# gevaertlab/sequoia-pub

Hardware: AMD Instinct MI355X
Metric: slides/sec (1000-patch WSI, UNI-dim, 20k-gene head) (higher is better)
Workload: dtype f16x3; 1 GPU; pipeline: 1000 x 224x224 uint8 patches/slide -> ResNet-50 embed -> k-Means(100) -> ViS(D=2048, depth 6, 16 heads, G=20820) forward (BASELINE config 3), patches uploaded from pinned host memory every step; embedder=ResNet-50 (src/resnet.py forward_extract), feature_dim=2048, patch_size=224, parallelism=slide-sharded x1

## Files before the change

### sequoia-pub_amd/csrc/chain_x3.hip

```cpp
#include "gemm.h"
#include "x3_fmt.h"

#include <cstdio>
#include <cstdlib>
#include <type_traits>

extern int g_dbg;

namespace {

constexpr uint32_t OOB = 0x80000000u;
typedef __attribute__((address_space(3))) void lds_void;

__device__ __forceinline__ void glds16(__amdgpu_buffer_rsrc_t rsrc, char* lds_base, uint32_t voffset) {
    __builtin_amdgcn_raw_ptr_buffer_load_lds(rsrc, (lds_void*)lds_base, 16, voffset, 0, 0, 0);
}
__device__ __forceinline__ u32x4 lds128(const char* p) { return *reinterpret_cast<const u32x4*>(p); }
template <int N> __device__ __forceinline__ void wait_vm() { asm volatile("s_waitcnt vmcnt(%0)" ::"n"(N) : "memory"); }
__device__ __forceinline__ void wait_vm_n(int n) {
    switch (n) {
        case 0: wait_vm<0>(); break;
        case 2: wait_vm<2>(); break;
        case 4: wait_vm<4>(); break;
        case 6: wait_vm<6>(); break;
// ... 11 lines not shown
constexpr int B_PLANE = N1 * 64;
constexpr int KT_BYTES = 2 * A_PLANE + 2 * B_PLANE;
constexpr int LDS_BYTES = 2 * KT_BYTES;
constexpr int YROW = N1 * 4;

struct ChainX3Args {
    const uint16_t* t2; long long plT2;
    const uint16_t* w3; const uint16_t* w1n; long long plW;
    const float* b3; const float* cs3; const float* b1n; const float* cs1n;
    const uint16_t* res; long long plRes;
    uint16_t* y; long long plY;
    uint16_t* t1n; long long plT1n;
    int P;
    uint32_t t2_bytes, w3_bytes;
    const uint16_t* xin; long long plX;
    const uint16_t* wd;
    const float* bd; const float* csd;
    uint32_t wd_bytes;
    const uint16_t* t1; long long plT1;
    const uint16_t* w2;
    const float* b2; const float* cs2;
    uint32_t w2_bytes;
    int W, HW;
    int dbg;
    int xcd_walk;
};

template <int N2, bool F16, bool DS, bool TAIL, bool WIDE = false>
__global__ __launch_bounds__(256, 2) void chain_x3_kernel(const ChainX3Args p) {
    using Fmt = X3Fmt<F16>;
    extern __shared__ __attribute__((aligned(16))) char smem[];
    const int tid = threadIdx.x, lane = tid & 63;
    const int wave = __builtin_amdgcn_readfirstlane(tid >> 6);
    const int l31 = lane & 31, lh = lane >> 5;

    const auto rsTh = __builtin_amdgcn_make_buffer_rsrc((void*)p.t2, 0, (int)p.t2_bytes, 0x00020000);
    const auto rsTl = __builtin_amdgcn_make_buffer_rsrc((void*)(p.t2 + p.plT2), 0, (int)p.t2_bytes, 0x00020000);
    const auto rsXh = __builtin_amdgcn_make_buffer_rsrc((void*)(DS ? p.xin : p.t2), 0, (int)p.t2_bytes, 0x00020000);
    const auto rsXl = __builtin_amdgcn_make_buffer_rsrc((void*)(DS ? p.xin + p.plX : p.t2 + p.plT2), 0, (int)p.t2_bytes, 0x00020000);

    constexpr int NI2 = N2 == 64 ? 1 : 2;
    const int pi = N2 == 64 ? wave >> 1 : 0, cj = N2 == 64 ? wave & 1 : wave;
    const uint16_t* const w1src = p.w1n + (size_t)cj * 16 * 512 + lane * 8;
    constexpr int W1PRE = DS ? 4 : 3;
    u32x4 wbh[4][4], wbl[4][4];
    auto load_w1 = [&](int g, int slot) {
// ... 231 lines not shown
                    const uint32_t h = Fmt::pack2(d0, d1);
                    const uint32_t l = Fmt::rest2(d0, d1, h);
                    acc[i][j][r] = x3_relu((s3 * acc[i][j][r] + b3) + Fmt::sum_lo(h, l));
                    acc[i][j][r + 1] = x3_relu((s3 * acc[i][j][r + 1] + b3) + Fmt::sum_hi(h, l));
                }
        }
    }
    __syncthreads();

#pragma unroll
    for (int i = 0; i < 2; ++i)
#pragma unroll
        for (int j = 0; j < 2; ++j)
#pragma unroll
            for (int r = 0; r < 16; ++r) {
                const int row = i * 32 + (r & 3) + 8 * (r >> 2) + 4 * lh;
                const int col = wave * 64 + j * 32 + l31;
                *reinterpret_cast<float*>(smem + row * YROW + ((((col >> 3) ^ (row & 31))) << 5) + (col & 7) * 4) = acc[i][j][r];
            }
#pragma unroll
    for (int g = 0; g < W1PRE; ++g) load_w1(g, g);
    __syncthreads();
    {
#pragma unroll
        for (int u = 0; u < 8; ++u) {
            const int row = u * 8 + rsub;
            const int m = p0 + row;
            char* chunk = smem + row * YROW + ((c8 ^ (row & 31)) << 5);
            const f32x4 a0 = *reinterpret_cast<const f32x4*>(chunk), a1 = *reinterpret_cast<const f32x4*>(chunk + 16);
            float v[8] = {a0[0], a0[1], a0[2], a0[3], a1[0], a1[1], a1[2], a1[3]};
            if constexpr (!DS) {
                float idn[8];
                x3_join8<F16>(rh[u], rl[u], idn);
#pragma unroll
                for (int e = 0; e < 8; ++e) v[e] = x3_relu((scale8[e] * v[e] + bias8[e]) + idn[e]);
            }
            u32x4 hi, lo;
            x3_split8<F16>(v, hi, lo);
            *reinterpret_cast<u32x4*>(chunk) = hi;
            *reinterpret_cast<u32x4*>(chunk + 16) = lo;
            if (m < p.P && !(p.dbg & 1)) {
                u32x4* qh = reinterpret_cast<u32x4*>(p.y + (size_t)m * N1 + c8 * 8);
                u32x4* ql = reinterpret_cast<u32x4*>(p.y + p.plY + (size_t)m * N1 + c8 * 8);
                *qh = hi; *ql = lo;
            }
        }
    }
    __syncthreads();

    f32x16 acc2[NI2];
#pragma unroll
    for (int i = 0; i < NI2; ++i)
#pragma unroll
        for (int e = 0; e < 16; ++e) acc2[i][e] = 0.f;
    if (!(p.dbg & 8))
#pragma unroll
    for (int g = 0; g < 4; ++g) {
        if (g == 0)
#pragma unroll
            for (int g2 = W1PRE; g2 < 4; ++g2) load_w1(g2, g2);
#pragma unroll
        for (int s4 = 0; s4 < 4; ++s4) {
            const int s = g * 4 + s4;
            u32x4 ah[NI2], al[NI2];
#pragma unroll
            for (int i = 0; i < NI2; ++i) {
// ... 62 lines not shown
        const bool d = e0 >= FRAG_WD;
        const int r = e0 - (d ? FRAG_WD : 0), q = r >> 9, lane = (r & 511) >> 3;
        const uint16_t* w = d ? wd : w3;
        if (w) src = at(w, (q >> 2) * 32 + (lane & 31), (q & 3) * 16 + (lane >> 5) * 8, N1, K1);
    } else if (e0 < FRAG_WD) {
        const int r = e0 - FRAG_W1, q = r >> 9, lane = (r & 511) >> 3;
        if ((q >> 4) * 32 < n2) src = at(w1n, (q >> 4) * 32 + (lane & 31), (q & 15) * 16 + (lane >> 5) * 8, n2, N1);
    } else if (w2) {
        const int r = e0 - FRAG_W2, g = r >> 11, n = (r & 2047) >> 5, kk = r & 31;
        const int cb = g / 9, tap = g - cb * 9;
        src = at(w2, n, tap * 64 + cb * 32 + kk, 64, 576);
    }
    if (src) *reinterpret_cast<u32x4*>(dst + (size_t)pl * FRAG + e0) = *reinterpret_cast<const u32x4*>(src + (size_t)pl * plSrc);
}

}

size_t sq_chain_x3_frag_bytes() { return (size_t)2 * FRAG * 2; }

int sq_launch_chain_x3_c64(int f16, const uint16_t* t2, long long plT2, const uint16_t* res, long long plRes, uint16_t* y, long long plY,
                           uint16_t* t1n, long long plT1n, int n2, const uint16_t* w3, const uint16_t* w1n, long long plW, size_t w3_bytes,
                           const float* b3, const float* cs3, const float* b1n, const float* cs1n,
                           const uint16_t* xin, long long plX, const uint16_t* wd, size_t wd_bytes, const float* bd, const float* csd,
                           const uint16_t* t1, long long plT1, const uint16_t* w2, size_t w2_bytes, const float* b2, const float* cs2, int W, int HW,
                           long long P, uint16_t* frag, int w_tiled, hipStream_t stream) {
    SQ_REQUIRE(n2 == 64 || n2 == 128, "chain_x3: next width %d (64 or 128)", n2);
    SQ_REQUIRE(P > 0 && P * N1 * 2 < (1ll << 31), "chain_x3: %lld pixels exceed the 2 GiB descriptor limit", P);
    const bool tail = t1 != nullptr;
    SQ_REQUIRE((t2 || tail) && y && t1n && w3 && w1n && b3 && b1n && frag && w3_bytes >= (size_t)N1 * K1 * 2, "chain_x3: null pointer / weight extent");
    SQ_REQUIRE(!tail || (w2 && b2 && w2_bytes >= (size_t)64 * 576 * 2 && W >= 3 && W <= 70 && HW >= W && HW % W == 0 && P % HW == 0),
               "chain_x3: tail form needs the 3x3 weights and maps up to 70 wide (W=%d, HW=%d)", W, HW);
    const bool wide = tail && W > 62;
    const bool ds = res == nullptr;
    SQ_REQUIRE(!ds || (xin && wd && bd && wd_bytes >= (size_t)N1 * K1 * 2), "chain_x3: neither an identity tensor nor a downsample branch");
    ChainX3Args a;
    hipLaunchKernelGGL(chain_x3_pack_kernel, dim3((2 * (FRAG / 8) + 255) / 256), dim3(256), 0, stream, w3, w1n, ds ? wd : nullptr,
                       tail ? w2 : nullptr, plW, n2, w_tiled, frag);
    SQ_LAUNCH_CHECK();
    a.t2 = t2; a.plT2 = plT2; a.w3 = frag; a.w1n = frag + FRAG_W1; a.plW = FRAG; a.b3 = b3; a.cs3 = cs3; a.b1n = b1n; a.cs1n = cs1n;
    a.res = res; a.plRes = plRes; a.y = y; a.plY = plY; a.t1n = t1n; a.plT1n = plT1n; a.P = (int)P;
    a.t2_bytes = (uint32_t)(P * K1 * 2);
    auto clamp = [](size_t b) { return (uint32_t)(b < 0x7fffffffu ? b : 0x7fffffffu); };
    a.w3_bytes = clamp(w3_bytes);
    a.xin = xin; a.plX = plX; a.wd = frag + FRAG_WD; a.bd = bd; a.csd = csd; a.wd_bytes = clamp(wd_bytes);
    a.t1 = t1; a.plT1 = plT1; a.w2 = frag + FRAG_W2; a.b2 = b2; a.cs2 = cs2; a.w2_bytes = (uint32_t)((FRAG - FRAG_W2) * 2); a.W = W; a.HW = HW; a.dbg = g_dbg;
    { const char* e = getenv("SQ_X3_TAIL_XCD_WALK"); a.xcd_walk = tail ? (e ? atoi(e) : 64) : 0; }
    using I64 = std::integral_constant<int, 64>; using I128 = std::integral_constant<int, 128>;
    using T = std::true_type; using F = std::false_type;
    auto pick_tail = [&](auto n2c, auto f16c, auto dsc) {
        return wide ? (const void*)chain_x3_kernel<decltype(n2c)::value, decltype(f16c)::value, decltype(dsc)::value, true, true>
             : tail ? (const void*)chain_x3_kernel<decltype(n2c)::value, decltype(f16c)::value, decltype(dsc)::value, true>
                    : (const void*)chain_x3_kernel<decltype(n2c)::value, decltype(f16c)::value, decltype(dsc)::value, false>;
    };
    auto pick_ds = [&](auto n2c, auto f16c) { return ds ? pick_tail(n2c, f16c, T{}) : pick_tail(n2c, f16c, F{}); };
    auto pick_f16 = [&](auto n2c) { return f16 ? pick_ds(n2c, T{}) : pick_ds(n2c, F{}); };
    const void* fn = n2 == 64 ? pick_f16(I64{}) : pick_f16(I128{});
    SQ_HIP_CHECK(hipFuncSetAttribute(fn, hipFuncAttributeMaxDynamicSharedMemorySize, LDS_BYTES));
    int prof = -1;
    if (sq_prof_on()) {
        char name[96];
        snprintf(name, sizeof(name), "%s_%s_c64_cn%d%s_P%lld", tail ? "tail" : "chain", f16 ? "f16x3" : "bf16x3", n2, ds ? "_ds" : "", P);
        prof = sq_prof_begin(name, 2.0 * P * ((tail ? 576.0 * 64 : 0.0) + 64.0 * 256 * (ds ? 2 : 1) + 256.0 * n2), (double)P * 4.0 * (64 + (ds ? 64 : 256) + 256 + n2), stream);
    }
    const dim3 grid((unsigned)((P + PX - 1) / PX)), block(256);
    void* kargs[] = {(void*)&a};
    SQ_HIP_CHECK(hipLaunchKernel(fn, grid, block, kargs, LDS_BYTES, stream));
    if (prof >= 0) sq_prof_end(prof, stream);
    return SQ_OK;
}

extern "C" int sq_dbg_chain_x3(int f16, int n2, int ds, int tail, long long P, int W, void* act, void* wts, void* fp, void* frag, void* stream) {
    uint16_t* a = (uint16_t*)act;
    const uint16_t* w = (const uint16_t*)wts;
    const float* f = (const float*)fp;
    uint16_t* t1 = a; uint16_t* res = t1 + 2 * P * 64; uint16_t* y = res + 2 * P * 256; uint16_t* t1n = y + 2 * P * 256;
    const long long plW = 102400;
    return sq_launch_chain_x3_c64(f16, tail ? nullptr : t1, P * 64, ds ? nullptr : res, P * 256, y, P * 256, t1n, P * 128, n2,
                                  w, w + 16384, plW, (size_t)(plW * 2), f, f + 256, f + 512, f + 640,
                                  ds ? t1 : nullptr, P * 64, ds ? w + 49152 : nullptr, (size_t)(plW - 49152) * 2, ds ? f + 768 : nullptr, ds ? f + 1024 : nullptr,
                                  tail ? t1 : nullptr, P * 64, tail ? w + 65536 : nullptr, (size_t)(plW - 65536) * 2, tail ? f + 1280 : nullptr,
                                  tail ? f + 1344 : nullptr, W, W * W, P, (uint16_t*)frag, 0, (hipStream_t)stream);
}
```

### sequoia-pub_amd/csrc/chain_x3w.hip

```cpp
#include "gemm.h"
#include "x3_fmt.h"

#include <cstdio>
#include <cstdlib>
#include <type_traits>

extern int g_dbg;

namespace {

constexpr uint32_t OOB = 0x80000000u;
typedef __attribute__((address_space(3))) void lds_void;

__device__ __forceinline__ void glds16(__amdgpu_buffer_rsrc_t rsrc, char* lds_base, uint32_t voffset) {
    __builtin_amdgcn_raw_ptr_buffer_load_lds(rsrc, (lds_void*)lds_base, 16, voffset, 0, 0, 0);
}
__device__ __forceinline__ void glds16_nt(__amdgpu_buffer_rsrc_t rsrc, char* lds_base, uint32_t voffset) {
    __builtin_amdgcn_raw_ptr_buffer_load_lds(rsrc, (lds_void*)lds_base, 16, voffset, 0, 0, 2);
}
__device__ __forceinline__ u32x4 lds128(const char* p) { return *reinterpret_cast<const u32x4*>(p); }
__device__ __forceinline__ u32x2 lds64(const char* p) { return *reinterpret_cast<const u32x2*>(p); }
__device__ __forceinline__ void st_lds64(char* p, u32x2 v) { *reinterpret_cast<u32x2*>(p) = v; }
template <int N> __device__ __forceinline__ void wait_vm() { asm volatile("s_waitcnt vmcnt(%0)" ::"n"(N) : "memory"); }
__device__ __forceinline__ void wait_vm_n(int n) {
    switch (n >> 1) {
        case 0: wait_vm<0>(); break;
        case 1: wait_vm<2>(); break;
        case 2: wait_vm<4>(); break;
        case 3: wait_vm<6>(); break;
        case 4: wait_vm<8>(); break;
        case 5: wait_vm<10>(); break;
        case 6: wait_vm<12>(); break;
        case 7: wait_vm<14>(); break;
        default: wait_vm<16>(); break;
    }
}

struct ChainWArgs {
    const uint16_t* t2; long long plT2;
    const uint16_t* res; long long plRes;
    uint16_t* y; long long plY;
    uint16_t* t1n; long long plT1n;
    const uint16_t* w3; const uint16_t* w1n; long long plW;
    const float* b3; const float* cs3; const float* b1n; const float* cs1n;
    int P, tiles, tiled;
    uint32_t w3_bytes, w1n_bytes;
    int dbg;
};

template <int C, int N2_> struct ChainWCfg {
    static constexpr int N2 = N2_, N1 = 4 * C, NS = N1 / 32, KS1 = C / 16, NT2 = N2 / 32;
    static constexpr int H = N2 / 128;
    static constexpr int KSH = KS1 / H;
    static constexpr int KTL = C / H / 32;
    static constexpr int W3R = KTL / 2;
    static constexpr int NW3 = 2 * W3R;
    static constexpr int STEPS = H * NS + H;
    static constexpr int T = 512, PX = 128;
    static constexpr int UNIT = 16384, UH = 8192;
    static constexpr int RING = 6 * UNIT;
    static constexpr int XYW = 4096;
    static constexpr int XY = 4 * 3 * XYW;
    static constexpr int BIAS_FLOATS = 2 * N1 + 2 * N2;
    static constexpr int LDS_BYTES = RING + XY + BIAS_FLOATS * 4;
    static_assert((C == 128 && (N2 == 128 || N2 == 256)) || (C == 256 && N2 == 256), "C -> next width: 128 -> 128 | 256 (28 x 28 stage), 256 -> 256 (14 x 14 stage)");
    static_assert(32 * (C / H) * 4 <= UNIT && N2 * (32 / H) * 4 == UNIT && KTL >= 2, "unit sizes");
    static_assert(32 * N2 * 2 * 4 <= RING, "t1' staging (one plane per pixel group) must fit the dead ring");
};
// ... 169 lines not shown
#pragma unroll
                    for (int g = 0; g < 4; ++g) {
                        char* a = xrow + ((g ^ swz) << 4) + 8 * lh;
                        const int cb = s * 32 + 8 * g + 4 * lh;
                        const f32x4 b = *reinterpret_cast<const f32x4*>(BS + cb), sc = *reinterpret_cast<const f32x4*>(BS + N1 + cb);
                        const u32x2 ih = lds64(a), il = lds64(a + 2048);
                        float v[4];
                        v[0] = x3_relu((sc[0] * accy[4 * g + 0] + b[0]) + Fmt::sum_lo(ih[0], il[0]));
                        v[1] = x3_relu((sc[1] * accy[4 * g + 1] + b[1]) + Fmt::sum_hi(ih[0], il[0]));
                        v[2] = x3_relu((sc[2] * accy[4 * g + 2] + b[2]) + Fmt::sum_lo(ih[1], il[1]));
                        v[3] = x3_relu((sc[3] * accy[4 * g + 3] + b[3]) + Fmt::sum_hi(ih[1], il[1]));
                        const uint32_t h0 = Fmt::pack2(v[0], v[1]), h1 = Fmt::pack2(v[2], v[3]);
                        const uint32_t l0 = Fmt::rest2(v[0], v[1], h0);
                        const uint32_t l1 = Fmt::rest2(v[2], v[3], h1);
                        st_lds64(a, u32x2{h0, h1});
                        st_lds64(a + 2048, u32x2{l0, l1});
                    }
                }
                asm volatile("s_waitcnt lgkmcnt(0)" ::: "memory");
                __builtin_amdgcn_s_barrier();
            }
        }
    } else {
        const uint32_t act_bytes = (uint32_t)p.P * N1 * 2u;
        const auto rsYh = __builtin_amdgcn_make_buffer_rsrc((void*)p.y, 0, (int)act_bytes, 0x00020000);
        const auto rsYl = __builtin_amdgcn_make_buffer_rsrc((void*)(p.y + p.plY), 0, (int)act_bytes, 0x00020000);
        const auto rsTh = __builtin_amdgcn_make_buffer_rsrc((void*)p.t1n, 0, (int)((uint32_t)p.P * N2 * 2u), 0x00020000);
        const auto rsTl = __builtin_amdgcn_make_buffer_rsrc((void*)(p.t1n + p.plT1n), 0, (int)((uint32_t)p.P * N2 * 2u), 0x00020000);
        f32x16 acc2[NT2];
#pragma unroll
        for (int i = 0; i < NT2; ++i)
#pragma unroll
            for (int e = 0; e < 16; ++e) acc2[i][e] = 0.f;
        asm volatile("s_waitcnt vmcnt(0) lgkmcnt(0)" ::: "memory");
        __builtin_amdgcn_s_barrier();
#pragma unroll
        for (int h = 0; h < H; ++h) __builtin_amdgcn_s_barrier();
        for (int s = 0; s < NS; ++s) {
            const char* xy = myXY + (s % 3) * XYW;
#pragma unroll
            for (int h = 0; h < H; ++h) {
                const int i = (s + 1) * H + h;
                const bool st = h == 0 && !(dbg & 1) && (H == 1 || (s & 1));
                constexpr int NSP = H == 1 ? 4 : 8;
                u32x4 sv[4];
                auto store_off = [&](int r) -> uint32_t {
                    if constexpr (H == 1) {
                        const int e = (r >> 1) * 64 + lane, row = e >> 2, cl = (e & 3) ^ ((row >> 2) & 3);
                        const int pr = p0 + row;
                        return pr < p.P ? ((uint32_t)pr * N1 + (uint32_t)(s * 32 + cl * 8)) * 2u : OOB;
                    } else {
                        const int row = (r & 3) * 8 + (lane >> 3), c8 = lane & 7;
                        const int pr = p0 + row;
                        return pr < p.P ? ((uint32_t)pr * N1 + (uint32_t)((s - 1) * 32 + c8 * 8)) * 2u : OOB;
                    }
                };
                auto store_read = [&](int r) {
                    if (!st) return;
                    if constexpr (H == 1) {
                        const int e = (r >> 1) * 64 + lane;
                        sv[r & 3] = lds128(xy + (r & 1) * 2048 + e * 16);
                    } else {
                        const int row = (r & 3) * 8 + (lane >> 3), c8 = lane & 7;
                        const char* img = myXY + ((c8 >> 2) ? s % 3 : (s - 1) % 3) * XYW;
                        sv[r & 3] = lds128(img + (r >> 2) * 2048 + row * 64 + (((c8 & 3) ^ ((row >> 2) & 3)) << 4));
                    }
                };
                auto store_piece = [&](int r) {
                    if (!st) return;
                    const bool lo = H == 1 ? (r & 1) : (r >> 2);
                    if (nt) {
                        if (lo) __builtin_amdgcn_raw_buffer_store_b128(sv[r & 3], rsYl, store_off(r), 0, 2);
                        else __builtin_amdgcn_raw_buffer_store_b128(sv[r & 3], rsYh, store_off(r), 0, 2);
                    } else {
                        if (lo) __builtin_amdgcn_raw_buffer_store_b128(sv[r & 3], rsYl, store_off(r), 0, 0);
                        else __builtin_amdgcn_raw_buffer_store_b128(sv[r & 3], rsYh, store_off(r), 0, 0);
                    }
// ... 101 lines not shown
}

template <int C, int N2, bool F16>
int launch_chainw(const ChainWArgs& a, hipStream_t stream) {
    using Cfg = ChainWCfg<C, N2>;
    static SqDevOnce attr;
    if (attr.needed()) {
        SQ_HIP_CHECK(hipFuncSetAttribute((const void*)chain_x3w_kernel<C, N2, F16, false>, hipFuncAttributeMaxDynamicSharedMemorySize, Cfg::LDS_BYTES));
        SQ_HIP_CHECK(hipFuncSetAttribute((const void*)chain_x3w_kernel<C, N2, F16, true>, hipFuncAttributeMaxDynamicSharedMemorySize, Cfg::LDS_BYTES));
        attr.done();
    }
    if (a.dbg) hipLaunchKernelGGL((chain_x3w_kernel<C, N2, F16, true>), dim3(a.tiles), dim3(Cfg::T), Cfg::LDS_BYTES, stream, a);
    else hipLaunchKernelGGL((chain_x3w_kernel<C, N2, F16, false>), dim3(a.tiles), dim3(Cfg::T), Cfg::LDS_BYTES, stream, a);
    SQ_LAUNCH_CHECK();
    return SQ_OK;
}

}

bool sq_chain_x3w_eligible(int c, int n2) { return (c == 128 && (n2 == 128 || n2 == 256)) || (c == 256 && n2 == 256); }

int sq_launch_chain_x3w(int f16, int c, const uint16_t* t2, long long plT2, const uint16_t* res, long long plRes, uint16_t* y, long long plY,
                        uint16_t* t1n, long long plT1n, int n2, const uint16_t* w3, const uint16_t* w1n, long long plW, size_t w3_bytes, size_t w1n_bytes,
                        const float* b3, const float* cs3, const float* b1n, const float* cs1n, long long P, int w_tiled, hipStream_t stream) {
    SQ_REQUIRE(sq_chain_x3w_eligible(c, n2), "chain_x3w: C=%d next width %d (128 -> 128 | 256, 256 -> 256)", c, n2);
    SQ_REQUIRE(P > 0 && P * 4 * c * 2 < (1ll << 31), "chain_x3w: %lld pixels exceed the 2 GiB descriptor limit", P);
    SQ_REQUIRE(t2 && res && y && t1n && w3 && w1n && b3 && b1n, "chain_x3w: null pointer");
    SQ_REQUIRE(w3_bytes >= (size_t)4 * c * c * 2 && w1n_bytes >= (size_t)n2 * 4 * c * 2, "chain_x3w: weight extents");
    SQ_REQUIRE((((uintptr_t)t2 | (uintptr_t)res | (uintptr_t)y | (uintptr_t)t1n | (uintptr_t)w3 | (uintptr_t)w1n) & 15) == 0 &&
               ((plT2 | plRes | plY | plT1n | plW) & 7) == 0, "chain_x3w: planes must be 16-byte aligned");
    ChainWArgs a;
    a.t2 = t2; a.plT2 = plT2; a.res = res; a.plRes = plRes; a.y = y; a.plY = plY; a.t1n = t1n; a.plT1n = plT1n;
    a.w3 = w3; a.w1n = w1n; a.plW = plW; a.b3 = b3; a.cs3 = cs3; a.b1n = b1n; a.cs1n = cs1n;
    a.P = (int)P; a.tiled = w_tiled; a.dbg = g_dbg;
    auto clamp = [](size_t b) { return (uint32_t)(b < 0x7fffffffu ? b : 0x7fffffffu); };
    a.w3_bytes = clamp(w3_bytes); a.w1n_bytes = clamp(w1n_bytes);
    a.tiles = (int)((P + 127) / 128);
    int prof = -1;
    if (sq_prof_on()) {
        char name[96];
        snprintf(name, sizeof(name), "chainw_%s_c%d_cn%d_P%lld", f16 ? "f16x3" : "bf16x3", c, n2, P);
        prof = sq_prof_begin(name, 2.0 * P * (4.0 * c * c + 4.0 * c * n2), (double)P * 4.0 * (c + 4 * c + 4 * c + n2), stream);
    }
    int rc;
    if (c == 256) rc = f16 ? launch_chainw<256, 256, true>(a, stream) : launch_chainw<256, 256, false>(a, stream);
    else if (n2 == 256) rc = f16 ? launch_chainw<128, 256, true>(a, stream) : launch_chainw<128, 256, false>(a, stream);
    else rc = f16 ? launch_chainw<128, 128, true>(a, stream) : launch_chainw<128, 128, false>(a, stream);
    if (prof >= 0) sq_prof_end(prof, stream);
    return rc;
}

extern "C" int sq_dbg_chain_x3w(int f16, int c, int n2, long long P, const void* t2_hi, const void* t2_lo, const void* res_hi, const void* res_lo,
                                void* y_hi, void* y_lo, void* t1n_hi, void* t1n_lo, const void* w3_hi, const void* w3_lo,
                                const void* w1n_hi, const void* w1n_lo, const float* b3, const float* cs3, const float* b1n, const float* cs1n,
                                int w_tiled, void* stream) {
    const uint16_t* t2 = (const uint16_t*)t2_hi; const uint16_t* res = (const uint16_t*)res_hi;
    uint16_t* y = (uint16_t*)y_hi; uint16_t* t1n = (uint16_t*)t1n_hi;
    const uint16_t* w3 = (const uint16_t*)w3_hi; const uint16_t* w1 = (const uint16_t*)w1n_hi;
    const long long plW = (const uint16_t*)w3_lo - w3;
    SQ_REQUIRE((const uint16_t*)w1n_lo - w1 == plW, "dbg_chain_x3w: both weights must share the plane distance");
    const size_t w3b = (size_t)4 * c * c * 2, w1b = (size_t)n2 * 4 * c * 2;
    return sq_launch_chain_x3w(f16, c, t2, (const uint16_t*)t2_lo - t2, res, (const uint16_t*)res_lo - res, y, (uint16_t*)y_lo - y, t1n, (uint16_t*)t1n_lo - t1n,
                               n2, w3, w1, plW, w3b, w1b, b3, cs3, b1n, cs1n, P, w_tiled, (hipStream_t)stream);
}
```

### sequoia-pub_amd/csrc/resnet.hip

```cpp
#include "../../include/sequoia_hip.h"
#include "gemm.h"
#include "x3_fmt.h"

int sq_launch_bottleneck_tail_c64(const bf16_t* t1, const bf16_t* res, bf16_t* y, bf16_t* t1n, int cn,
                                  const bf16_t* w2, const bf16_t* w3, const bf16_t* w1n, size_t w2_bytes, size_t w3_bytes, size_t w1n_bytes,
                                  const float* b2, const float* b3, const float* b1n,
                                  const bf16_t* xin, const bf16_t* wd, size_t wd_bytes, const float* bd,
                                  int n_img, int H, int W, hipStream_t stream);
int sq_launch_bottleneck_chain_c256(const bf16_t* t2, const bf16_t* res, bf16_t* y, bf16_t* t1n, const bf16_t* w3,
                                    const bf16_t* w1n, size_t w3_bytes, size_t w1n_bytes, const float* b3, const float* b1n,
                                    long long P, hipStream_t stream);
int sq_launch_bottleneck_chain_c128(const bf16_t* t2, const bf16_t* res, bf16_t* y, bf16_t* t1n, int cn, const bf16_t* w3,
                                    const bf16_t* w1n, size_t w3_bytes, size_t w1n_bytes, const float* b3, const float* b1n,
                                    long long P, hipStream_t stream);
int sq_launch_conv1_pool_bf16(const uint8_t* u8, const float* f32_nchw, const bf16_t* w152, const float* bias, bf16_t* out,
                              int n, int H, int W, hipStream_t stream);
int sq_launch_chain_x3_c64(int f16, const uint16_t* t2, long long plT2, const uint16_t* res, long long plRes, uint16_t* y, long long plY,
                           uint16_t* t1n, long long plT1n, int n2, const uint16_t* w3, const uint16_t* w1n, long long plW, size_t w3_bytes,
                           const float* b3, const float* cs3, const float* b1n, const float* cs1n,
                           const uint16_t* xin, long long plX, const uint16_t* wd, size_t wd_bytes, const float* bd, const float* csd,
                           const uint16_t* t1, long long plT1, const uint16_t* w2, size_t w2_bytes, const float* b2, const float* cs2, int W, int HW,
                           long long P, uint16_t* frag, int w_tiled, hipStream_t stream);
size_t sq_chain_x3_frag_bytes();
bool sq_chain_x3w_eligible(int c, int n2);
int sq_launch_chain_x3w(int f16, int c, const uint16_t* t2, long long plT2, const uint16_t* res, long long plRes, uint16_t* y, long long plY,
                        uint16_t* t1n, long long plT1n, int n2, const uint16_t* w3, const uint16_t* w1n, long long plW, size_t w3_bytes, size_t w1n_bytes,
                        const float* b3, const float* cs3, const float* b1n, const float* cs1n, long long P, int w_tiled, hipStream_t stream);
int sq_launch_conv1_pool_x3(int f16, const uint8_t* u8, const float* f32_nchw, const uint16_t* w152_hi, long long w_plane, const float* bias,
                            const float* colscale, uint16_t* out_hi, long long out_plane, int n, int H, int W, hipStream_t stream,
                            const uint16_t* w1_hi, int w1_tiled, const float* b1, const float* cs1, uint16_t* t1_hi);

namespace {

constexpr int CONV1_K = 147, CONV1_KP = 152;
constexpr float BN_MEAN[3] = {0.485f, 0.456f, 0.406f};
constexpr float BN_STD[3] = {0.229f, 0.224f, 0.225f};

template <typename T>
__global__ __launch_bounds__(256) void im2col_conv1_kernel(const uint8_t* __restrict__ src_u8, const float* __restrict__ src_f32,
                                                           T* __restrict__ out, int n, int H, int W, int OH, int OW) {
    __shared__ float lut[3][256];
    __shared__ int8_t t_kh[CONV1_KP], t_kw[CONV1_KP], t_c[CONV1_KP];
    for (int i = threadIdx.x; i < 3 * 256; i += 256) {
        const int c = i >> 8, v = i & 255;
        const float p = (float)v / 255.0f;
        lut[c][v] = (p - BN_MEAN[c]) / BN_STD[c];
    }
    for (int k = threadIdx.x; k < CONV1_KP; k += 256) {
        const int tap = k / 3;
        t_c[k] = k < CONV1_K ? (int8_t)(k - tap * 3) : (int8_t)-1;
// ... 297 lines not shown
            hipLaunchKernelGGL(im2col_conv1_kernel<float>, dim3((int)nb), dim3(256), 0, st, patches_u8, patches_f32_nchw, (float*)b.col, n, H0, W0, OH1, OW1);
            SQ_LAUNCH_CHECK();
            GemmArgs g;
            const sq_conv_desc& d = lay.conv[0];
            g.M = n * OH1 * OW1; g.N = 64; g.K = CONV1_KP;
            g.A = b.col; g.lda = CONV1_KP; g.a_bytes = (size_t)g.M * CONV1_KP * es;
            g.B = W(d); g.ldb = CONV1_KP; g.b_bytes = w_bytes_total;
            g.bias = bias + d.b_off; g.act = SQ_ACT_RELU;
            g.C = b.act[0]; g.ldc = 64; g.out_dtype = dtype;
            RUN(sq_launch_gemm(g, dtype, st));
        }
        {
            const size_t work = (size_t)n * H * Wd * 64 / (16 / es);
            size_t nb = (work + 255) / 256; if (nb > 65535) nb = 65535;
            hipLaunchKernelGGL(maxpool3x3s2_kernel<float>, dim3((int)nb), dim3(256), 0, st, (const float*)b.act[0], (float*)b.act[1], n, OH1, OW1, H, Wd, 64);
            SQ_LAUNCH_CHECK();
        }
    }
    const bool fuse56 = lp && !sq_env_flag("SQ_RESNET_NO_FUSE") && (128 + 2 * Wd + 2) * 128 <= 32768;
    const bool fuse_chain = lp && !sq_env_flag("SQ_RESNET_NO_FUSE") && !sq_env_flag("SQ_RESNET_NO_CHAIN");
    const bool fuse_chain256 = fuse_chain;
    int xi = 1, ci = 1, t1i = stem_t1 ? 2 : -1;
    const int blocks[4] = {3, 4, 6, 3};
    for (int li = 0; li < 4; ++li)
        for (int bk = 0; bk < blocks[li]; ++bk) {
            int free_[4], nf = 0;
            for (int i = 0; i < 5; ++i) if (i != xi && i != t1i) free_[nf++] = i;
            void* x = b.act[xi];
            const int t1_idx = t1i >= 0 ? t1i : free_[--nf];
            void* t1 = b.act[t1_idx];
            const sq_conv_desc& c1 = lay.conv[ci]; const sq_conv_desc& c2 = lay.conv[ci + 1]; const sq_conv_desc& c3 = lay.conv[ci + 2];
            const bool has_ds = bk == 0;
            const int OH = (H - 1) / c2.stride + 1, OW = (Wd - 1) / c2.stride + 1;
            if (t1i < 0) RUN(conv(c1, x, H, Wd, t1, H, Wd, nullptr, SQ_ACT_RELU));
            const int cnext = ci + (has_ds ? 4 : 3);
            if (fuse56 && li == 0) {
                void* y = b.act[free_[1]]; void* t1n = b.act[free_[2]];
                const sq_conv_desc& n1 = lay.conv[cnext];
                const sq_conv_desc& dsd = lay.conv[ci + 3];
                auto rest = [&](const sq_conv_desc& d) { return w_bytes_total - (size_t)d.w_off * es; };
                RUN(sq_launch_bottleneck_tail_c64((const bf16_t*)t1, has_ds ? nullptr : (const bf16_t*)x, (bf16_t*)y, (bf16_t*)t1n, n1.cout,
                                                  (const bf16_t*)W(c2), (const bf16_t*)W(c3), (const bf16_t*)W(n1), rest(c2), rest(c3), rest(n1),
                                                  bias + c2.b_off, bias + c3.b_off, bias + n1.b_off,
                                                  has_ds ? (const bf16_t*)x : nullptr, has_ds ? (const bf16_t*)W(dsd) : nullptr,
                                                  has_ds ? rest(dsd) : 0, has_ds ? bias + dsd.b_off : nullptr, n, H, Wd, st));
                xi = free_[1];
                t1i = free_[2];
                ci = cnext;
                continue;
            }
            void* t2 = b.act[free_[0]]; void* ds = b.act[free_[1]]; void* y = b.act[free_[2]];
            const bool x3_chain = x3 && !sq_env_flag("SQ_RESNET_NO_CHAIN") && c3.cin == 64 && c3.cout == 256 && c2.stride == 1 &&
                cnext < SQ_RESNET50_CONVS && lay.conv[cnext].k == 1 && lay.conv[cnext].stride == 1 && lay.conv[cnext].cin == 256 &&
                (lay.conv[cnext].cout == 64 || lay.conv[cnext].cout == 128) &&
                (!has_ds || (lay.conv[ci + 3].k == 1 && lay.conv[ci + 3].stride == 1 && lay.conv[ci + 3].cin == 64 && !sq_env_flag("SQ_RESNET_NO_CHAIN_DS")));
            const bool x3_tail = x3_chain && c2.k == 3 && c2.cin == 64 && c2.cout == 64 && Wd <= 70 && !sq_env_flag("SQ_RESNET_NO_TAIL");
            if (!x3_tail) RUN(conv(c2, t1, H, Wd, t2, OH, OW, nullptr, SQ_ACT_RELU));
            if (x3_chain) {
                const sq_conv_desc& n1 = lay.conv[cnext];
                const sq_conv_desc& dsd = lay.conv[ci + 3];
                auto rest = [&](const sq_conv_desc& d) { return w_bytes_total - (size_t)d.w_off * es; };
                void* t1n = x3_tail ? t2 : t1;
                RUN(sq_launch_chain_x3_c64(f16, x3_tail ? nullptr : (const uint16_t*)t2, act_plane, has_ds ? nullptr : (const uint16_t*)x, act_plane,
                                           (uint16_t*)y, act_plane, (uint16_t*)t1n, act_plane, n1.cout, (const uint16_t*)W(c3), (const uint16_t*)W(n1),
                                           lay.w_total, rest(c3), bias + c3.b_off, colscale + c3.b_off, bias + n1.b_off, colscale + n1.b_off,
                                           has_ds ? (const uint16_t*)x : nullptr, act_plane, has_ds ? (const uint16_t*)W(dsd) : nullptr,
                                           has_ds ? rest(dsd) : 0, has_ds ? bias + dsd.b_off : nullptr, has_ds ? colscale + dsd.b_off : nullptr,
                                           x3_tail ? (const uint16_t*)t1 : nullptr, act_plane, x3_tail ? (const uint16_t*)W(c2) : nullptr,
                                           x3_tail ? rest(c2) : 0, x3_tail ? bias + c2.b_off : nullptr, x3_tail ? colscale + c2.b_off : nullptr, Wd, H * Wd,
                                           (long long)n * OH * OW, (uint16_t*)b.frag, 1, st));
                ci = cnext;
                xi = free_[2];
                t1i = x3_tail ? free_[0] : t1_idx;
                H = OH; Wd = OW;
                continue;
            }
            if (x3 && !has_ds && !sq_env_flag("SQ_RESNET_NO_CHAINW") && c3.k == 1 && c3.cout == 4 * c3.cin && cnext < SQ_RESNET50_CONVS &&
                lay.conv[cnext].k == 1 && lay.conv[cnext].stride == 1 && lay.conv[cnext].cin == c3.cout &&
                sq_chain_x3w_eligible(c3.cin, lay.conv[cnext].cout)) {
                const sq_conv_desc& n1 = lay.conv[cnext];
                auto rest = [&](const sq_conv_desc& d) { return w_bytes_total - (size_t)d.w_off * es; };
                RUN(sq_launch_chain_x3w(f16, c3.cin, (const uint16_t*)t2, act_plane, (const uint16_t*)x, act_plane, (uint16_t*)y, act_plane,
                                        (uint16_t*)t1, act_plane, n1.cout, (const uint16_t*)W(c3), (const uint16_t*)W(n1), lay.w_total, rest(c3), rest(n1),
                                        bias + c3.b_off, colscale + c3.b_off, bias + n1.b_off, colscale + n1.b_off, (long long)n * OH * OW, 1, st));
                ci = cnext;
                xi = free_[2];
                t1i = t1_idx;
                H = OH; Wd = OW;
                continue;
            }
            const void* identity = x;
            const bool x3_dual = x3 && has_ds && lay.conv[ci + 3].k == 1 && c3.k == 1 && c3.cout % 128 == 0 && !sq_env_flag("SQ_RESNET_NO_DUAL");
            if (has_ds && !x3_dual) {
                RUN(conv(lay.conv[ci + 3], x, H, Wd, ds, OH, OW, nullptr, SQ_ACT_NONE));
                identity = ds;
            }
            if (fuse_chain && c3.cin == 128 && c3.cout == 512 && cnext < SQ_RESNET50_CONVS && lay.conv[cnext].k == 1 &&
                lay.conv[cnext].cin == 512 && (lay.conv[cnext].cout == 128 || lay.conv[cnext].cout == 256)) {
                const sq_conv_desc& n1 = lay.conv[cnext];
                auto rest = [&](const sq_conv_desc& d) { return w_bytes_total - (size_t)d.w_off * es; };
                RUN(sq_launch_bottleneck_chain_c128((const bf16_t*)t2, (const bf16_t*)identity, (bf16_t*)y, (bf16_t*)t1, n1.cout,
                                                    (const bf16_t*)W(c3), (const bf16_t*)W(n1), rest(c3), rest(n1), bias + c3.b_off,
                                                    bias + n1.b_off, (long long)n * OH * OW, st));
                ci = cnext;
                xi = free_[2];
                t1i = t1_idx;
                H = OH; Wd = OW;
                continue;
            }
            if (fuse_chain256 && c3.cin == 256 && c3.cout == 1024 && cnext < SQ_RESNET50_CONVS && lay.conv[cnext].k == 1 &&
                lay.conv[cnext].cin == 1024 && lay.conv[cnext].cout == 256) {
                const sq_conv_desc& n1 = lay.conv[cnext];
                auto rest = [&](const sq_conv_desc& d) { return w_bytes_total - (size_t)d.w_off * es; };
                RUN(sq_launch_bottleneck_chain_c256((const bf16_t*)t2, (const bf16_t*)identity, (bf16_t*)y, (bf16_t*)t1,
                                                    (const bf16_t*)W(c3), (const bf16_t*)W(n1), rest(c3), rest(n1), bias + c3.b_off,
                                                    bias + n1.b_off, (long long)n * OH * OW, st));
                ci = cnext;
                xi = free_[2];
                t1i = t1_idx;
                H = OH; Wd = OW;
                continue;
            }
            if (x3_dual) RUN(conv(c3, t2, OH, OW, y, OH, OW, nullptr, SQ_ACT_RELU, &lay.conv[ci + 3], x, H, Wd));
            else RUN(conv(c3, t2, OH, OW, y, OH, OW, identity, SQ_ACT_RELU));
            ci = cnext;
            xi = free_[2];
            t1i = -1;
            H = OH; Wd = OW;
        }
    {
        const int total = n * 2048;
        if (f16) hipLaunchKernelGGL(avgpool7_x3_kernel<true>, dim3((total + 255) / 256), dim3(256), 0, st, (const bf16_t*)b.act[xi], act_plane, features, n, H, Wd, 2048, nonfinite_flag);
        else if (x3) hipLaunchKernelGGL(avgpool7_x3_kernel<false>, dim3((total + 255) / 256), dim3(256), 0, st, (const bf16_t*)b.act[xi], act_plane, features, n, H, Wd, 2048, nonfinite_flag);
        else if (lp) hipLaunchKernelGGL(avgpool7_kernel<bf16_t>, dim3((total + 255) / 256), dim3(256), 0, st, (const bf16_t*)b.act[xi], features, n, H, Wd, 2048);
        else hipLaunchKernelGGL(avgpool7_kernel<float>, dim3((total + 255) / 256), dim3(256), 0, st, (const float*)b.act[xi], features, n, H, Wd, 2048);
        SQ_LAUNCH_CHECK();
    }
#undef RUN
    (void)act_cap;
    return SQ_OK;
}
```

Before: 34.77 slides/s.

## Store only strided-subsampled stage outputs consumed by next stage's downsample

For the last bottleneck block of stages 1-3, the fused chain kernels now write the block output y only at positions the next stage's stride-2 1x1 downsample will read, compacted into a subsampled map. The following downsample conv then runs with stride 1 on the pre-subsampled map. This cuts the global store traffic for the final block of each stage and the strided gather in the downsample, at the cost of per-row index arithmetic and a tighter coupling between blocks. The old behaviour can be restored with the SQ_RESNET_STORE_ALL flag.

```diff
diff --git a/sequoia-pub_amd/csrc/chain_x3.hip b/sequoia-pub_amd/csrc/chain_x3.hip
--- a/sequoia-pub_amd/csrc/chain_x3.hip
+++ b/sequoia-pub_amd/csrc/chain_x3.hip
@@ -1,5 +1,6 @@
 #include "gemm.h"
 #include "x3_fmt.h"
+#include "x3_sub.h"
 
 #include <cstdio>
 #include <cstdlib>
@@ -57,6 +58,7 @@
     const float* b2; const float* cs2;
     uint32_t w2_bytes;
     int W, HW;
+    int H, y_stride;
     int dbg;
     int xcd_walk;
 };
@@ -334,6 +336,8 @@
     for (int g = 0; g < W1PRE; ++g) load_w1(g, g);
     __syncthreads();
     {
+        X3SubPos sub(p.H, p.W, p.y_stride);
+        if (p.y_stride > 1) sub.seek(p0 + rsub);
 #pragma unroll
         for (int u = 0; u < 8; ++u) {
             const int row = u * 8 + rsub;
@@ -351,9 +355,16 @@
             x3_split8<F16>(v, hi, lo);
             *reinterpret_cast<u32x4*>(chunk) = hi;
             *reinterpret_cast<u32x4*>(chunk + 16) = lo;
-            if (m < p.P && !(p.dbg & 1)) {
-                u32x4* qh = reinterpret_cast<u32x4*>(p.y + (size_t)m * N1 + c8 * 8);
-                u32x4* ql = reinterpret_cast<u32x4*>(p.y + p.plY + (size_t)m * N1 + c8 * 8);
+            bool keep = m < p.P && !(p.dbg & 1);
+            size_t yrow = (size_t)m;
+            if (p.y_stride > 1) {
+                keep = keep && sub.kept();
+                yrow = (size_t)sub.row();
+                sub.step(8);
+            }
+            if (keep) {
+                u32x4* qh = reinterpret_cast<u32x4*>(p.y + yrow * N1 + c8 * 8);
+                u32x4* ql = reinterpret_cast<u32x4*>(p.y + p.plY + yrow * N1 + c8 * 8);
                 *qh = hi; *ql = lo;
             }
         }
@@ -462,14 +473,17 @@
                            uint16_t* t1n, long long plT1n, int n2, const uint16_t* w3, const uint16_t* w1n, long long plW, size_t w3_bytes,
                            const float* b3, const float* cs3, const float* b1n, const float* cs1n,
                            const uint16_t* xin, long long plX, const uint16_t* wd, size_t wd_bytes, const float* bd, const float* csd,
-                           const uint16_t* t1, long long plT1, const uint16_t* w2, size_t w2_bytes, const float* b2, const float* cs2, int W, int HW,
-                           long long P, uint16_t* frag, int w_tiled, hipStream_t stream) {
+                           const uint16_t* t1, long long plT1, const uint16_t* w2, size_t w2_bytes, const float* b2, const float* cs2, int H, int W, int HW,
+                           int y_stride, long long P, uint16_t* frag, int w_tiled, hipStream_t stream) {
     SQ_REQUIRE(n2 == 64 || n2 == 128, "chain_x3: next width %d (64 or 128)", n2);
     SQ_REQUIRE(P > 0 && P * N1 * 2 < (1ll << 31), "chain_x3: %lld pixels exceed the 2 GiB descriptor limit", P);
     const bool tail = t1 != nullptr;
     SQ_REQUIRE((t2 || tail) && y && t1n && w3 && w1n && b3 && b1n && frag && w3_bytes >= (size_t)N1 * K1 * 2, "chain_x3: null pointer / weight extent");
     SQ_REQUIRE(!tail || (w2 && b2 && w2_bytes >= (size_t)64 * 576 * 2 && W >= 3 && W <= 70 && HW >= W && HW % W == 0 && P % HW == 0),
                "chain_x3: tail form needs the 3x3 weights and maps up to 70 wide (W=%d, HW=%d)", W, HW);
+    SQ_REQUIRE(y_stride >= 1 && (y_stride == 1 || (H >= 1 && W >= 1 && HW == (long long)H * W && P % HW == 0)) && (!tail || HW == (long long)H * W),
+               "chain_x3: map geometry H=%d W=%d HW=%d y_stride=%d for %lld pixels", H, W, HW, y_stride, P);
+    const long long y_rows = y_stride > 1 ? P / HW * ((H - 1) / y_stride + 1) * ((W - 1) / y_stride + 1) : P;
     const bool wide = tail && W > 62;
     const bool ds = res == nullptr;
     SQ_REQUIRE(!ds || (xin && wd && bd && wd_bytes >= (size_t)N1 * K1 * 2), "chain_x3: neither an identity tensor nor a downsample branch");
@@ -483,7 +497,7 @@
     auto clamp = [](size_t b) { return (uint32_t)(b < 0x7fffffffu ? b : 0x7fffffffu); };
     a.w3_bytes = clamp(w3_bytes);
     a.xin = xin; a.plX = plX; a.wd = frag + FRAG_WD; a.bd = bd; a.csd = csd; a.wd_bytes = clamp(wd_bytes);
-    a.t1 = t1; a.plT1 = plT1; a.w2 = frag + FRAG_W2; a.b2 = b2; a.cs2 = cs2; a.w2_bytes = (uint32_t)((FRAG - FRAG_W2) * 2); a.W = W; a.HW = HW; a.dbg = g_dbg;
+    a.t1 = t1; a.plT1 = plT1; a.w2 = frag + FRAG_W2; a.b2 = b2; a.cs2 = cs2; a.w2_bytes = (uint32_t)((FRAG - FRAG_W2) * 2); a.W = W; a.HW = HW; a.H = H; a.y_stride = y_stride; a.dbg = g_dbg;
     { const char* e = getenv("SQ_X3_TAIL_XCD_WALK"); a.xcd_walk = tail ? (e ? atoi(e) : 64) : 0; }
     using I64 = std::integral_constant<int, 64>; using I128 = std::integral_constant<int, 128>;
     using T = std::true_type; using F = std::false_type;
@@ -500,7 +514,7 @@
     if (sq_prof_on()) {
         char name[96];
         snprintf(name, sizeof(name), "%s_%s_c64_cn%d%s_P%lld", tail ? "tail" : "chain", f16 ? "f16x3" : "bf16x3", n2, ds ? "_ds" : "", P);
-        prof = sq_prof_begin(name, 2.0 * P * ((tail ? 576.0 * 64 : 0.0) + 64.0 * 256 * (ds ? 2 : 1) + 256.0 * n2), (double)P * 4.0 * (64 + (ds ? 64 : 256) + 256 + n2), stream);
+        prof = sq_prof_begin(name, 2.0 * P * ((tail ? 576.0 * 64 : 0.0) + 64.0 * 256 * (ds ? 2 : 1) + 256.0 * n2), ((double)P * (64 + (ds ? 64 : 256) + n2) + (double)y_rows * 256) * 4.0, stream);
     }
     const dim3 grid((unsigned)((P + PX - 1) / PX)), block(256);
     void* kargs[] = {(void*)&a};
@@ -519,5 +533,31 @@
                                   w, w + 16384, plW, (size_t)(plW * 2), f, f + 256, f + 512, f + 640,
                                   ds ? t1 : nullptr, P * 64, ds ? w + 49152 : nullptr, (size_t)(plW - 49152) * 2, ds ? f + 768 : nullptr, ds ? f + 1024 : nullptr,
                                   tail ? t1 : nullptr, P * 64, tail ? w + 65536 : nullptr, (size_t)(plW - 65536) * 2, tail ? f + 1280 : nullptr,
-                                  tail ? f + 1344 : nullptr, W, W * W, P, (uint16_t*)frag, 0, (hipStream_t)stream);
-}
+                                  tail ? f + 1344 : nullptr, W, W, W * W, 1, P, (uint16_t*)frag, 0, (hipStream_t)stream);
+}
+
+extern "C" int sq_dbg_chain_x3_sub(int f16, int n2, int ds, int tail, long long P, int W, void* act, void* wts, void* fp, void* frag, void* stream,
+                                   int H, int stride) {
+    uint16_t* a = (uint16_t*)act;
+    const uint16_t* w = (const uint16_t*)wts;
+    const float* f = (const float*)fp;
+    uint16_t* t1 = a; uint16_t* res = t1 + 2 * P * 64; uint16_t* y = res + 2 * P * 256; uint16_t* t1n = y + 2 * P * 256;
+    const long long plW = 102400;
+    return sq_launch_chain_x3_c64(f16, tail ? nullptr : t1, P * 64, ds ? nullptr : res, P * 256, y, P * 256, t1n, P * 128, n2,
+                                  w, w + 16384, plW, (size_t)(plW * 2), f, f + 256, f + 512, f + 640,
+                                  ds ? t1 : nullptr, P * 64, ds ? w + 49152 : nullptr, (size_t)(plW - 49152) * 2, ds ? f + 768 : nullptr, ds ? f + 1024 : nullptr,
+                                  tail ? t1 : nullptr, P * 64, tail ? w + 65536 : nullptr, (size_t)(plW - 65536) * 2, tail ? f + 1280 : nullptr,
+                                  tail ? f + 1344 : nullptr, H, W, H * W, stride, P, (uint16_t*)frag, 0, (hipStream_t)stream);
+}
+
+extern "C" int sq_dbg_x3_sub_index(int H, int W, int s, long long m, long long* row) {
+    int r = 0;
+    const bool kept = x3_sub_index(H, W, s, m, &r);
+    *row = r;
+    return kept ? 1 : 0;
+}
+extern "C" void sq_dbg_x3_sub_walk(int H, int W, int s, long long m0, int step, int count, long long* rows) {
+    X3SubPos q(H, W, s);
+    q.seek(m0);
+    for (int i = 0; i < count; ++i) { rows[i] = q.kept() ? q.row() : -1; q.step(step); }
+}
diff --git a/sequoia-pub_amd/csrc/chain_x3w.hip b/sequoia-pub_amd/csrc/chain_x3w.hip
--- a/sequoia-pub_amd/csrc/chain_x3w.hip
+++ b/sequoia-pub_amd/csrc/chain_x3w.hip
@@ -1,5 +1,6 @@
 #include "gemm.h"
 #include "x3_fmt.h"
+#include "x3_sub.h"
 
 #include <cstdio>
 #include <cstdlib>
@@ -44,6 +45,7 @@
     const uint16_t* w3; const uint16_t* w1n; long long plW;
     const float* b3; const float* cs3; const float* b1n; const float* cs1n;
     int P, tiles, tiled;
+    int H, W, y_stride, y_rows;
     uint32_t w3_bytes, w1n_bytes;
     int dbg;
 };
@@ -259,9 +261,19 @@
             }
         }
     } else {
-        const uint32_t act_bytes = (uint32_t)p.P * N1 * 2u;
-        const auto rsYh = __builtin_amdgcn_make_buffer_rsrc((void*)p.y, 0, (int)act_bytes, 0x00020000);
-        const auto rsYl = __builtin_amdgcn_make_buffer_rsrc((void*)(p.y + p.plY), 0, (int)act_bytes, 0x00020000);
+        const uint32_t y_bytes = (uint32_t)p.y_rows * N1 * 2u;
+        const auto rsYh = __builtin_amdgcn_make_buffer_rsrc((void*)p.y, 0, (int)y_bytes, 0x00020000);
+        const auto rsYl = __builtin_amdgcn_make_buffer_rsrc((void*)(p.y + p.plY), 0, (int)y_bytes, 0x00020000);
+        constexpr int NYR = H == 1 ? 2 : 4;
+        uint32_t ybase[NYR];
+#pragma unroll
+        for (int q = 0; q < NYR; ++q) {
+            const int pr = p0 + (H == 1 ? (q * 64 + lane) >> 2 : q * 8 + (lane >> 3));
+            int yr = pr;
+            bool keep = pr < p.P;
+            if (p.y_stride > 1) keep = x3_sub_index(p.H, p.W, p.y_stride, pr, &yr) && keep;
+            ybase[q] = keep ? (uint32_t)yr * (uint32_t)(N1 * 2) : OOB;
+        }
         const auto rsTh = __builtin_amdgcn_make_buffer_rsrc((void*)p.t1n, 0, (int)((uint32_t)p.P * N2 * 2u), 0x00020000);
         const auto rsTl = __builtin_amdgcn_make_buffer_rsrc((void*)(p.t1n + p.plT1n), 0, (int)((uint32_t)p.P * N2 * 2u), 0x00020000);
         f32x16 acc2[NT2];
@@ -284,12 +296,10 @@
                 auto store_off = [&](int r) -> uint32_t {
                     if constexpr (H == 1) {
                         const int e = (r >> 1) * 64 + lane, row = e >> 2, cl = (e & 3) ^ ((row >> 2) & 3);
-                        const int pr = p0 + row;
-                        return pr < p.P ? ((uint32_t)pr * N1 + (uint32_t)(s * 32 + cl * 8)) * 2u : OOB;
+                        return ybase[r >> 1] + (uint32_t)(s * 32 + cl * 8) * 2u;
                     } else {
-                        const int row = (r & 3) * 8 + (lane >> 3), c8 = lane & 7;
-                        const int pr = p0 + row;
-                        return pr < p.P ? ((uint32_t)pr * N1 + (uint32_t)((s - 1) * 32 + c8 * 8)) * 2u : OOB;
+                        const int c8 = lane & 7;
+                        return ybase[r & 3] + (uint32_t)((s - 1) * 32 + c8 * 8) * 2u;
                     }
                 };
                 auto store_read = [&](int r) {
@@ -437,14 +447,19 @@
 
 int sq_launch_chain_x3w(int f16, int c, const uint16_t* t2, long long plT2, const uint16_t* res, long long plRes, uint16_t* y, long long plY,
                         uint16_t* t1n, long long plT1n, int n2, const uint16_t* w3, const uint16_t* w1n, long long plW, size_t w3_bytes, size_t w1n_bytes,
-                        const float* b3, const float* cs3, const float* b1n, const float* cs1n, long long P, int w_tiled, hipStream_t stream) {
+                        const float* b3, const float* cs3, const float* b1n, const float* cs1n, int H, int W, int y_stride, long long P, int w_tiled,
+                        hipStream_t stream) {
     SQ_REQUIRE(sq_chain_x3w_eligible(c, n2), "chain_x3w: C=%d next width %d (128 -> 128 | 256, 256 -> 256)", c, n2);
     SQ_REQUIRE(P > 0 && P * 4 * c * 2 < (1ll << 31), "chain_x3w: %lld pixels exceed the 2 GiB descriptor limit", P);
     SQ_REQUIRE(t2 && res && y && t1n && w3 && w1n && b3 && b1n, "chain_x3w: null pointer");
     SQ_REQUIRE(w3_bytes >= (size_t)4 * c * c * 2 && w1n_bytes >= (size_t)n2 * 4 * c * 2, "chain_x3w: weight extents");
     SQ_REQUIRE((((uintptr_t)t2 | (uintptr_t)res | (uintptr_t)y | (uintptr_t)t1n | (uintptr_t)w3 | (uintptr_t)w1n) & 15) == 0 &&
                ((plT2 | plRes | plY | plT1n | plW) & 7) == 0, "chain_x3w: planes must be 16-byte aligned");
+    SQ_REQUIRE(y_stride >= 1 && (y_stride == 1 || (H >= 1 && W >= 1 && P % ((long long)H * W) == 0)),
+               "chain_x3w: map geometry H=%d W=%d y_stride=%d for %lld pixels", H, W, y_stride, P);
+    const long long y_rows = y_stride > 1 ? P / ((long long)H * W) * ((H - 1) / y_stride + 1) * ((W - 1) / y_stride + 1) : P;
     ChainWArgs a;
+    a.H = H; a.W = W; a.y_stride = y_stride; a.y_rows = (int)y_rows;
     a.t2 = t2; a.plT2 = plT2; a.res = res; a.plRes = plRes; a.y = y; a.plY = plY; a.t1n = t1n; a.plT1n = plT1n;
     a.w3 = w3; a.w1n = w1n; a.plW = plW; a.b3 = b3; a.cs3 = cs3; a.b1n = b1n; a.cs1n = cs1n;
     a.P = (int)P; a.tiled = w_tiled; a.dbg = g_dbg;
@@ -455,7 +470,7 @@
     if (sq_prof_on()) {
         char name[96];
         snprintf(name, sizeof(name), "chainw_%s_c%d_cn%d_P%lld", f16 ? "f16x3" : "bf16x3", c, n2, P);
-        prof = sq_prof_begin(name, 2.0 * P * (4.0 * c * c + 4.0 * c * n2), (double)P * 4.0 * (c + 4 * c + 4 * c + n2), stream);
+        prof = sq_prof_begin(name, 2.0 * P * (4.0 * c * c + 4.0 * c * n2), ((double)P * (c + 4 * c + n2) + (double)y_rows * 4 * c) * 4.0, stream);
     }
     int rc;
     if (c == 256) rc = f16 ? launch_chainw<256, 256, true>(a, stream) : launch_chainw<256, 256, false>(a, stream);
@@ -476,5 +491,19 @@
     SQ_REQUIRE((const uint16_t*)w1n_lo - w1 == plW, "dbg_chain_x3w: both weights must share the plane distance");
     const size_t w3b = (size_t)4 * c * c * 2, w1b = (size_t)n2 * 4 * c * 2;
     return sq_launch_chain_x3w(f16, c, t2, (const uint16_t*)t2_lo - t2, res, (const uint16_t*)res_lo - res, y, (uint16_t*)y_lo - y, t1n, (uint16_t*)t1n_lo - t1n,
-                               n2, w3, w1, plW, w3b, w1b, b3, cs3, b1n, cs1n, P, w_tiled, (hipStream_t)stream);
-}
+                               n2, w3, w1, plW, w3b, w1b, b3, cs3, b1n, cs1n, 0, 0, 1, P, w_tiled, (hipStream_t)stream);
+}
+
+extern "C" int sq_dbg_chain_x3w_sub(int f16, int c, int n2, long long P, const void* t2_hi, const void* t2_lo, const void* res_hi, const void* res_lo,
+                                    void* y_hi, void* y_lo, void* t1n_hi, void* t1n_lo, const void* w3_hi, const void* w3_lo,
+                                    const void* w1n_hi, const void* w1n_lo, const float* b3, const float* cs3, const float* b1n, const float* cs1n,
+                                    int w_tiled, void* stream, int H, int W, int stride) {
+    const uint16_t* t2 = (const uint16_t*)t2_hi; const uint16_t* res = (const uint16_t*)res_hi;
+    uint16_t* y = (uint16_t*)y_hi; uint16_t* t1n = (uint16_t*)t1n_hi;
+    const uint16_t* w3 = (const uint16_t*)w3_hi; const uint16_t* w1 = (const uint16_t*)w1n_hi;
+    const long long plW = (const uint16_t*)w3_lo - w3;
+    SQ_REQUIRE((const uint16_t*)w1n_lo - w1 == plW, "dbg_chain_x3w_sub: both weights must share the plane distance");
+    const size_t w3b = (size_t)4 * c * c * 2, w1b = (size_t)n2 * 4 * c * 2;
+    return sq_launch_chain_x3w(f16, c, t2, (const uint16_t*)t2_lo - t2, res, (const uint16_t*)res_lo - res, y, (uint16_t*)y_lo - y, t1n, (uint16_t*)t1n_lo - t1n,
+                               n2, w3, w1, plW, w3b, w1b, b3, cs3, b1n, cs1n, H, W, stride, P, w_tiled, (hipStream_t)stream);
+}
diff --git a/sequoia-pub_amd/csrc/resnet.hip b/sequoia-pub_amd/csrc/resnet.hip
--- a/sequoia-pub_amd/csrc/resnet.hip
+++ b/sequoia-pub_amd/csrc/resnet.hip
@@ -19,13 +19,14 @@
                            uint16_t* t1n, long long plT1n, int n2, const uint16_t* w3, const uint16_t* w1n, long long plW, size_t w3_bytes,
                            const float* b3, const float* cs3, const float* b1n, const float* cs1n,
                            const uint16_t* xin, long long plX, const uint16_t* wd, size_t wd_bytes, const float* bd, const float* csd,
-                           const uint16_t* t1, long long plT1, const uint16_t* w2, size_t w2_bytes, const float* b2, const float* cs2, int W, int HW,
-                           long long P, uint16_t* frag, int w_tiled, hipStream_t stream);
+                           const uint16_t* t1, long long plT1, const uint16_t* w2, size_t w2_bytes, const float* b2, const float* cs2, int H, int W, int HW,
+                           int y_stride, long long P, uint16_t* frag, int w_tiled, hipStream_t stream);
 size_t sq_chain_x3_frag_bytes();
 bool sq_chain_x3w_eligible(int c, int n2);
 int sq_launch_chain_x3w(int f16, int c, const uint16_t* t2, long long plT2, const uint16_t* res, long long plRes, uint16_t* y, long long plY,
                         uint16_t* t1n, long long plT1n, int n2, const uint16_t* w3, const uint16_t* w1n, long long plW, size_t w3_bytes, size_t w1n_bytes,
-                        const float* b3, const float* cs3, const float* b1n, const float* cs1n, long long P, int w_tiled, hipStream_t stream);
+                        const float* b3, const float* cs3, const float* b1n, const float* cs1n, int H, int W, int y_stride, long long P, int w_tiled,
+                        hipStream_t stream);
 int sq_launch_conv1_pool_x3(int f16, const uint8_t* u8, const float* f32_nchw, const uint16_t* w152_hi, long long w_plane, const float* bias,
                             const float* colscale, uint16_t* out_hi, long long out_plane, int n, int H, int W, hipStream_t stream,
                             const uint16_t* w1_hi, int w1_tiled, const float* b1, const float* cs1, uint16_t* t1_hi);
@@ -369,6 +370,13 @@
     const bool fuse_chain256 = fuse_chain;
     int xi = 1, ci = 1, t1i = stem_t1 ? 2 : -1;
     const int blocks[4] = {3, 4, 6, 3};
+    const bool store_all = sq_env_flag("SQ_RESNET_STORE_ALL");
+    bool x_sub = false;
+    auto y_stride_of = [&](int li, int bk, int cnext) -> int {
+        if (store_all || li >= 3 || bk != blocks[li] - 1 || cnext + 3 >= SQ_RESNET50_CONVS) return 1;
+        const sq_conv_desc& n2 = lay.conv[cnext + 1]; const sq_conv_desc& nd = lay.conv[cnext + 3];
+        return nd.k == 1 && nd.pad == 0 && nd.stride > 1 && n2.stride == nd.stride ? nd.stride : 1;
+    };
     for (int li = 0; li < 4; ++li)
         for (int bk = 0; bk < blocks[li]; ++bk) {
             int free_[4], nf = 0;
@@ -378,6 +386,8 @@
             void* t1 = b.act[t1_idx];
             const sq_conv_desc& c1 = lay.conv[ci]; const sq_conv_desc& c2 = lay.conv[ci + 1]; const sq_conv_desc& c3 = lay.conv[ci + 2];
             const bool has_ds = bk == 0;
+            SQ_REQUIRE(!x_sub || (has_ds && t1i >= 0 && lay.conv[ci + 3].stride > 1),
+                       "resnet50: a strided stage output needs a strided downsample block with its reduce already computed");
             const int OH = (H - 1) / c2.stride + 1, OW = (Wd - 1) / c2.stride + 1;
             if (t1i < 0) RUN(conv(c1, x, H, Wd, t1, H, Wd, nullptr, SQ_ACT_RELU));
             const int cnext = ci + (has_ds ? 4 : 3);
@@ -414,8 +424,9 @@
                                            has_ds ? (const uint16_t*)x : nullptr, act_plane, has_ds ? (const uint16_t*)W(dsd) : nullptr,
                                            has_ds ? rest(dsd) : 0, has_ds ? bias + dsd.b_off : nullptr, has_ds ? colscale + dsd.b_off : nullptr,
                                            x3_tail ? (const uint16_t*)t1 : nullptr, act_plane, x3_tail ? (const uint16_t*)W(c2) : nullptr,
-                                           x3_tail ? rest(c2) : 0, x3_tail ? bias + c2.b_off : nullptr, x3_tail ? colscale + c2.b_off : nullptr, Wd, H * Wd,
-                                           (long long)n * OH * OW, (uint16_t*)b.frag, 1, st));
+                                           x3_tail ? rest(c2) : 0, x3_tail ? bias + c2.b_off : nullptr, x3_tail ? colscale + c2.b_off : nullptr, H, Wd, H * Wd,
+                                           y_stride_of(li, bk, cnext), (long long)n * OH * OW, (uint16_t*)b.frag, 1, st));
+                x_sub = y_stride_of(li, bk, cnext) > 1;
                 ci = cnext;
                 xi = free_[2];
                 t1i = x3_tail ? free_[0] : t1_idx;
@@ -429,7 +440,9 @@
                 auto rest = [&](const sq_conv_desc& d) { return w_bytes_total - (size_t)d.w_off * es; };
                 RUN(sq_launch_chain_x3w(f16, c3.cin, (const uint16_t*)t2, act_plane, (const uint16_t*)x, act_plane, (uint16_t*)y, act_plane,
                                         (uint16_t*)t1, act_plane, n1.cout, (const uint16_t*)W(c3), (const uint16_t*)W(n1), lay.w_total, rest(c3), rest(n1),
-                                        bias + c3.b_off, colscale + c3.b_off, bias + n1.b_off, colscale + n1.b_off, (long long)n * OH * OW, 1, st));
+                                        bias + c3.b_off, colscale + c3.b_off, bias + n1.b_off, colscale + n1.b_off, OH, OW, y_stride_of(li, bk, cnext),
+                                        (long long)n * OH * OW, 1, st));
+                x_sub = y_stride_of(li, bk, cnext) > 1;
                 ci = cnext;
                 xi = free_[2];
                 t1i = t1_idx;
@@ -437,9 +450,13 @@
                 continue;
             }
             const void* identity = x;
+            sq_conv_desc dsd1 = lay.conv[has_ds ? ci + 3 : ci];
+            const int dH = x_sub ? OH : H, dW = x_sub ? OW : Wd;
+            if (x_sub) dsd1.stride = 1;
+            x_sub = false;
             const bool x3_dual = x3 && has_ds && lay.conv[ci + 3].k == 1 && c3.k == 1 && c3.cout % 128 == 0 && !sq_env_flag("SQ_RESNET_NO_DUAL");
             if (has_ds && !x3_dual) {
-                RUN(conv(lay.conv[ci + 3], x, H, Wd, ds, OH, OW, nullptr, SQ_ACT_NONE));
+                RUN(conv(dsd1, x, dH, dW, ds, OH, OW, nullptr, SQ_ACT_NONE));
                 identity = ds;
             }
             if (fuse_chain && c3.cin == 128 && c3.cout == 512 && cnext < SQ_RESNET50_CONVS && lay.conv[cnext].k == 1 &&
@@ -468,7 +485,7 @@
                 H = OH; Wd = OW;
                 continue;
             }
-            if (x3_dual) RUN(conv(c3, t2, OH, OW, y, OH, OW, nullptr, SQ_ACT_RELU, &lay.conv[ci + 3], x, H, Wd));
+            if (x3_dual) RUN(conv(c3, t2, OH, OW, y, OH, OW, nullptr, SQ_ACT_RELU, &dsd1, x, dH, dW));
             else RUN(conv(c3, t2, OH, OW, y, OH, OW, identity, SQ_ACT_RELU));
             ci = cnext;
             xi = free_[2];
diff --git a/sequoia-pub_amd/csrc/x3_sub.h b/sequoia-pub_amd/csrc/x3_sub.h
--- /dev/null
+++ b/sequoia-pub_amd/csrc/x3_sub.h
@@ -0,0 +1,35 @@
+#pragma once
+#include <hip/hip_runtime.h>
+
+struct X3SubPos {
+    int H, W, s, OH, OW;
+    int img, h, w;
+    __host__ __device__ X3SubPos(int H_, int W_, int s_) : H(H_), W(W_), s(s_), OH((H_ - 1) / s_ + 1), OW((W_ - 1) / s_ + 1), img(0), h(0), w(0) {}
+    __host__ __device__ void seek(long long m) {
+        const unsigned hw = (unsigned)H * (unsigned)W;
+        img = (int)(m / hw);
+        const unsigned rem = (unsigned)(m - (long long)img * hw);
+        h = (int)(rem / (unsigned)W);
+        w = (int)(rem - (unsigned)h * (unsigned)W);
+    }
+    __host__ __device__ void step(int d) {
+        w += d;
+        while (w >= W) { w -= W; ++h; }
+        while (h >= H) { h -= H; ++img; }
+    }
+    __host__ __device__ bool kept() const {
+        if (s == 2) return ((h | w) & 1) == 0;
+        return h % s == 0 && w % s == 0;
+    }
+    __host__ __device__ int row() const {
+        if (s == 2) return (img * OH + (h >> 1)) * OW + (w >> 1);
+        return (img * OH + h / s) * OW + w / s;
+    }
+};
+
+__host__ __device__ inline bool x3_sub_index(int H, int W, int s, long long m, int* row) {
+    X3SubPos q(H, W, s);
+    q.seek(m);
+    *row = q.row();
+    return q.kept();
+}
```

After: 35.00 slides/s, median of 6. No clear change (+0.6%).
